# GuidoManni/BodySLAM

Hardware: AMD Instinct MI355X
Metric: frames/sec depth+pose+back-proj, 640x480 seq (higher is better)
Workload: dtype f16

## Files before the change

bodyslam_amd/_lib.py:

```python
from __future__ import annotations

import ctypes as C
import os
from typing import Optional

import torch

_HERE = os.path.dirname(os.path.abspath(__file__))
LIB_PATH = os.environ.get("BODYSLAM_HIP_LIB") or os.path.join(_HERE, "libbodyslam_hip.so")

F32, F16, BF16 = 0, 1, 2
F64 = 3
ACT_NONE, ACT_RELU, ACT_GELU, ACT_SOFTPLUS, ACT_SOFTPLUS_FAST = 0, 1, 2, 3, 4
OUT_PLAIN, OUT_SHUFFLE, OUT_QKV = 0, 1, 2

_TORCH2BS = {torch.float32: F32, torch.float16: F16, torch.bfloat16: BF16}
BS2TORCH = {F32: torch.float32, F16: torch.float16, BF16: torch.bfloat16}


class BodySlamHipError(RuntimeError):
    pass


class GemmDesc(C.Structure):
# ... 266 lines not shown
    if d.out_dtype == F32:
        per_row = [4.0, 4.0, 4.0]
    elif d.out_f8:
        per_row = [4.0, 3.0, 2.0]
    else:
        per_row = [2.0 * (2 if d.out_split_off else 1)] * 3
    full = float(d.M)
    r_planes = float(min(d.out_planes_rows, d.M)) if d.out_planes_rows else full
    r_lo = float(min(d.out_lo8_rows, d.M)) if d.out_lo8_rows else r_planes
    r_lo = min(r_lo, r_planes)
    out = d.N * (r_lo * per_row[0] + (r_planes - r_lo) * per_row[1] + (full - r_planes) * per_row[2])
    res = float(d.M) * d.N * (4 if (d.res and d.res_dtype == F32) else 0)
    return a + w + out + res


class Plan:

    def __init__(self, device=None):
        self.device = None if device is None else torch.device(device)
        self.calls = []
        self.names = []
        self.keep = []
        self.keep_descs = []
        self.marks = {}
        self.gemm_info = {}
        self.stack_info = {}
        self.events = None
        self._graph = None

    def gemm(self, name, A, W, out, **kw):
# ... 63 lines not shown
        if taps is None and self._graph is not None and not torch.cuda.is_current_stream_capturing():
            self._graph.replay()
            return
        st = torch.cuda.current_stream(self.device).cuda_stream
        if taps is None:
            for i, (fn, args) in enumerate(self.calls):
                rc = fn(*args, st)
                if rc:
                    check(rc, self.names[i])
            return
        means = taps.get("__site_means__")
        for i in range(len(self.calls) + 1):
            for (name, t, meta) in self.marks.get(i, []):
                if meta and meta[0] == "chanmean":
                    if means is not None:
                        _, off, M, lda, K = meta
                        means[name] = t.view(-1)[off: off + M * lda].view(M, lda)[:, :K].float().mean(0)
                    continue
                if means is None:
                    taps[name] = (t.clone(), meta)
            if i < len(self.calls):
                fn, args = self.calls[i]
                check(fn(*args, st), self.names[i])


_F8_ON_DEVICE = {}


def _f8_pack_device(device):
    if device is None or os.environ.get("BS_PACK_ON_HOST") == "1":
        return torch.device("cpu")
    device = torch.device(device)
# ... 340 lines not shown
```

bodyslam_amd/csrc/igemm.hip:

```cpp
#include <stdlib.h>

#include <map>
#include <mutex>
#include <utility>

#include "igemm_kernel.h"

namespace bs {

#define BS_DECL_TILE(t, cm)                                                  \
    int igemm_launch_tile##t##_f16_cm##cm(const IgemmParams&, bool, hipStream_t); \
    int igemm_launch_tile##t##_bf16_cm##cm(const IgemmParams&, bool, hipStream_t);
BS_DECL_TILE(1, 0) BS_DECL_TILE(1, 1)
BS_DECL_TILE(2, 0) BS_DECL_TILE(2, 1)
BS_DECL_TILE(3, 0) BS_DECL_TILE(3, 1)
BS_DECL_TILE(9, 0) BS_DECL_TILE(9, 1)
BS_DECL_TILE(10, 0) BS_DECL_TILE(11, 0)
BS_DECL_TILE(9s8, 0) BS_DECL_TILE(9s8, 1)
#undef BS_DECL_TILE

static int auto_tile(int M, int N, int K, int tile, bool conv) {
    if (tile != 0) return tile;
    if (N <= 32) return 3;
    if (N <= 64) return 2;
// ... 11 lines not shown
        default: BM = 128; BN = 128; break;
    }
}

static int launch_tile(IgemmParams& p, int dtype, bool conv, int tile, hipStream_t st) {
    int BM, BN;
    tile_dims(tile, BM, BN);
    p.ntm = cdiv(p.M - p.m_begin, BM);
    p.ntn = cdiv(p.N, BN);
    static const int strip_env = diag_env("BS_GEMM_STRIP") ? atoi(diag_env("BS_GEMM_STRIP")) : -1;
    const bool qkv = p.out_mode == BS_OUT_QKV;
    p.strip = conv ? 0 : (strip_env >= 0 ? strip_env : ((BM == 256 && BN == 256 && !qkv && p.ntn >= 8) ? 4 : 0));
    const int cm = (p.f8_stages > 0 || p.out_f8 || p.res_f8) ? 1 : 0;
    const bool h = dtype == BS_F16;
    const bool sched8 = tile == 9 && !(p.ablate & 32);
#define BS_TILE(t, c) (h ? igemm_launch_tile##t##_f16_cm##c(p, conv, st) : igemm_launch_tile##t##_bf16_cm##c(p, conv, st))
    switch (tile * 10 + cm) {
        case 10: return BS_TILE(1, 0);
        case 11: return BS_TILE(1, 1);
        case 20: return BS_TILE(2, 0);
        case 21: return BS_TILE(2, 1);
        case 30: return BS_TILE(3, 0);
        case 31: return BS_TILE(3, 1);
        case 90: return sched8 ? BS_TILE(9s8, 0) : BS_TILE(9, 0);
        case 91: return sched8 ? BS_TILE(9s8, 1) : BS_TILE(9, 1);
        case 100: return BS_TILE(10, 0);
        case 110: return BS_TILE(11, 0);
#undef BS_TILE
        default: set_error("bs_gemm: tile %d is not built for correction mode %d (tiles 1, 2, 3, 9, 10, 11)", tile, cm); return BS_ERR_INVALID;
    }
// ... 79 lines not shown
    BS_REQUIRE(d->lda % 8 == 0, "bs_gemm: lda=%d must be a multiple of 8 (16-byte rows)", d->lda);
    BS_REQUIRE(d->out_dtype == BS_F32 || d->out_dtype == d->dtype, "bs_gemm: out_dtype must be f32 or the operand dtype");
    BS_REQUIRE(!d->res || d->res_dtype == BS_F32 || d->res_dtype == d->dtype, "bs_gemm: res_dtype must be f32 or the operand dtype");
    IgemmParams p{};
    p.A = d->A; p.W = d->W; p.zero = zero_page();
    p.a_bytes = d->conv ? (long long)(d->M / (d->Hout > 0 && d->Wout > 0 ? d->Hout * d->Wout : 1)) * d->Hin * d->Win * d->lda * 2
                        : ((long long)(d->M - 1) * d->lda + (d->K + d->f8_seg / 2 - d->seg1)) * 2;
    BS_REQUIRE((long long)d->N * (d->K + d->f8_seg / 2) * 2 < 0x7FFFFFF0ll, "bs_gemm: weight matrix too large for one descriptor");
    p.M = d->M; p.N = d->N; p.K = d->K + d->f8_seg / 2; p.lda = d->lda;
    p.f8_seg = d->f8_seg;
    p.f8_sa0 = d->f8_scales & 0xff; p.f8_sb0 = (d->f8_scales >> 8) & 0xff; p.f8_sa1 = (d->f8_scales >> 16) & 0xff; p.f8_sb1 = d->f8_scales >> 24;
    p.out_f8 = d->out_f8;
    p.res_f8 = d->res_f8;
    BS_REQUIRE(!d->res_f8 || (d->res && d->res_dtype == d->dtype && d->res_split_off == 0 && d->ldr >= 2 * d->N && d->N % 8 == 0), "bs_gemm: res_f8 needs a 16-bit residual in (hi16 | hi8 | lo8) rows, ldr >= 2N");
    BS_REQUIRE(d->f8_seg >= 0 && d->f8_seg % 256 == 0, "bs_gemm: f8_seg=%d must be a multiple of 256 (two halves of whole 128-byte stages)", d->f8_seg);
    BS_REQUIRE(d->f8_seg == 0 || (d->seg1 == 0 && !d->relu_a), "bs_gemm: the FP8 segment excludes seg1 and relu_a");
    p.f8_stages = d->f8_seg / 128;
    BS_REQUIRE(d->out_f8 == 0 || (d->out_dtype == d->dtype && d->ldo % 8 == 0 &&
                                  ((d->out_mode == BS_OUT_PLAIN && d->out_split_off == d->N && d->N % 8 == 0) ||
                                   (d->out_mode == BS_OUT_SHUFFLE && d->out_split_off == d->shuffle_cout && d->shuffle_cout % 8 == 0))),
               "bs_gemm: out_f8 needs a plain / shuffle 16-bit output with out_split_off = channels, channels %% 8 == 0");
    p.Hin = d->Hin; p.Win = d->Win; p.Cin = d->Cin; p.Hout = d->Hout; p.Wout = d->Wout;
    p.KH = d->KH; p.KW = d->KW; p.stride = d->stride; p.pad_h = d->pad_h; p.pad_w = d->pad_w;
    if (d->conv) {
        BS_REQUIRE(d->Cin > 0 && d->Cin % 64 == 0, "bs_gemm: conv Cin=%d must be a multiple of 64", d->Cin);
        BS_REQUIRE(d->K == d->KH * d->KW * (d->Cin + d->seg1), "bs_gemm: conv K=%d != KH*KW*(Cin+seg1)", d->K);
        BS_REQUIRE(d->Hout > 0 && d->Wout > 0 && d->M % (d->Hout * d->Wout) == 0, "bs_gemm: conv M=%d not a multiple of Hout*Wout", d->M);
        BS_REQUIRE(d->stride > 0 && d->lda >= d->Cin, "bs_gemm: bad conv stride/lda");
        BS_REQUIRE(d->KH > 0 && d->KW > 0 && d->KH * d->KW <= 32, "bs_gemm: conv window %dx%d: at most 32 taps", d->KH, d->KW);
        BS_REQUIRE((long long)d->Hin * d->Win * d->lda * 2 * 4 < 0x7FFFFFF0ll, "bs_gemm: image too large for the 2 GiB tile window");
        p.tiles_per_tap = d->Cin / 64;
// ... 74 lines not shown
```

bodyslam_amd/csrc/igemm_kernel.h:

```cpp
#pragma once
#include <type_traits>

#include "common.h"

namespace bs {

struct IgemmParams {
    const void* A;
    const void* W;
    const void* zero;
    long long a_bytes;
    int M, N, K, lda;
    int Hin, Win, Cin, Hout, Wout, KH, KW, stride, pad_h, pad_w;
    int tiles_per_tap;
    int cin1;
    int split_off;
    int res_split_off;
    int relu_a;
    const float* bias;
    int bias_group_rows;
    int act;
    const float* scale;
    const void* res;
    const void* res2;
// ... 19 lines not shown
    int res_f8;
    int out_f8;
    int out2_relu;
    int out_lo8_rows;
    int f8_skip_from;
    int out_planes_rows;
    const float* bias2;
    int bias2_row0, bias2_group_rows;
    int strip;
    int ablate;
};

template <typename T>
__device__ __forceinline__ typename T16<T>::v8 relu8(typename T16<T>::v8 x) {
    typedef short s16x8 __attribute__((ext_vector_type(8)));
    s16x8 b = __builtin_bit_cast(s16x8, x);
    s16x8 neg = b >> 15;
    b = b & ~neg;
    return __builtin_bit_cast(typename T16<T>::v8, b);
}

template <typename T>
__device__ __forceinline__ void store4(void* base, int64_t off, int out_dtype, const float (&y)[4], int split_off = 0) {
    if (split_off > 0) {
        typename T16<T>::v4 h, l;
#pragma unroll
        for (int e = 0; e < 4; ++e) {
            h[e] = T16<T>::from_f32(y[e]);
            l[e] = T16<T>::from_f32(y[e] - T16<T>::to_f32(h[e]));
        }
        *reinterpret_cast<typename T16<T>::v4*>(reinterpret_cast<T*>(base) + off) = h;
        *reinterpret_cast<typename T16<T>::v4*>(reinterpret_cast<T*>(base) + off + split_off) = l;
        return;
    }
// ... 88 lines not shown
}

constexpr int NW_CHECK(int a, int b) { return a * b; }

template <int N>
__device__ __forceinline__ void wait_vmcnt() {
    asm volatile("s_waitcnt vmcnt(%0)" ::"n"(N) : "memory");
}

template <typename T, int BM, int BN, int WM, int WN, int BK, int STAGES, int MODE, bool PP = false, int CM = 0, int SCHED = 0>
__global__ __launch_bounds__(WM* WN * 64, 2) void igemm_kernel(const IgemmParams p) {
#if defined(__HIP_DEVICE_COMPILE__)
    constexpr bool CONV = MODE != 0;
    constexpr bool RELU_A = MODE == 2;
    constexpr bool F8 = CM != 0;
    constexpr int NT = WM * WN * 64;
    constexpr int ROWB = BK * 2;
    constexpr int LPR = ROWB / 16;
    constexpr int RPR = NT / LPR;
    constexpr int RPW = 64 / LPR;
    constexpr int RA = BM / RPR, RB = BN / RPR;
    static_assert(BK == 64 || BK == 32, "BK");
    static_assert(BM % RPR == 0 && BN % RPR == 0, "tile rows must be a multiple of the DMA round");
    constexpr int GL = RA + RB;
    static_assert(GL * (STAGES - 1) <= 63, "vmcnt range");
    constexpr int TM = BM / WM, TN = BN / WN;
    constexpr int FM = TM / 16, FN = TN / 16;
    static_assert(TM % 16 == 0 && TN % 16 == 0, "wave tile must be a multiple of 16");
    constexpr int A_BYTES = BM * ROWB, B_BYTES = BN * ROWB, STAGE = A_BYTES + B_BYTES;
    constexpr int LDS_BYTES = STAGES * STAGE;
// ... 221 lines not shown
                    for (int jj = 0; jj < 2; ++jj)
                        acc[ah * 4 + i][bh * 2 + jj] = __builtin_amdgcn_mfma_scale_f32_16x16x128_f8f6f4(op8(bf[bh][jj][0], bf[bh][jj][1]), a8,
                                                                                                        acc[ah * 4 + i][bh * 2 + jj], 0, 0, 0, scb, 0, sca);
                }
            } else {
#pragma unroll
                for (int kk = 0; kk < 2; ++kk)
#pragma unroll
                    for (int i = 0; i < 4; ++i)
#pragma unroll
                        for (int jj = 0; jj < 2; ++jj)
                            acc[ah * 4 + i][bh * 2 + jj] = T16<T>::mfma16(bf[bh][jj][kk], af[i][kk], acc[ah * 4 + i][bh * 2 + jj]);
            }
            __builtin_amdgcn_s_setprio(0);
        };
        auto relu_a = [&]() {
            if constexpr (RELU_A) {
#pragma unroll
                for (int i = 0; i < 4; ++i)
#pragma unroll
                    for (int kk = 0; kk < 2; ++kk) af[i][kk] = relu8<T>(af[i][kk]);
            }
        };
        auto tile = [&](int t, auto f8_tag, auto steady_tag) {
            constexpr bool F8S = decltype(f8_tag)::value == 1;
            constexpr bool STEADY = decltype(steady_tag)::value == 1;
            const int left = nt - 1 - t;
            const char* sa = smem + cbuf * STAGE;
            const char* sb = sa + A_BYTES;
            if constexpr (F8S) {
                const bool second = t >= nt16 + ((nt_all - nt16) >> 1);
                sca = (second ? p.f8_sa1 : p.f8_sa0) * 0x01010101;
                scb = (second ? p.f8_sb1 : p.f8_sb0) * 0x01010101;
            }
            read_w(sb, H0{});
            __builtin_amdgcn_sched_barrier(0);
            read_a(sa, 0);
            if ((STEADY || left >= 1) && dma) stage_piece(cbuf ^ 1, PW1{});
            if (STEADY || left >= 1) wait_vmcnt<8>();
            else wait_vmcnt<2>();
            phase_barrier();
            relu_a();
            multiply(f8_tag, H0{}, H0{});
            phase_barrier();
            read_w(sb, H1{});
            if (STEADY || left >= 1) {
                if (dma) stage_piece(cbuf ^ 1, PA1{});
                stage_advance();
                wait_vmcnt<8>();
            } else {
                wait_vmcnt<0>();
            }
            phase_barrier();
            multiply(f8_tag, H0{}, H1{});
            phase_barrier();
            read_a(sa, 1);
            if ((STEADY || left >= 2) && dma) stage_piece(cbuf, PA0{});
            phase_barrier();
            relu_a();
            multiply(f8_tag, H1{}, H1{});
            phase_barrier();
            if ((STEADY || left >= 2) && dma) stage_piece(cbuf, PW0{});
            if (STEADY || left >= 2) wait_vmcnt<8>();
            else if (left == 1) wait_vmcnt<4>();
            phase_barrier();
            multiply(f8_tag, H1{}, H0{});
            phase_barrier();
            cbuf ^= 1;
        };
        stage_piece(0, PA0{});
        stage_piece(0, PW0{});
        stage_piece(0, PW1{});
        stage_piece(0, PA1{});
        stage_advance();
// ... 1 lines not shown
            stage_piece(1, PA0{});
            stage_piece(1, PW0{});
            wait_vmcnt<8>();
        } else {
            wait_vmcnt<4>();
        }
        __builtin_amdgcn_s_waitcnt(0xc07f);
        phase_barrier();
        if (wm == 1) phase_barrier();
        using S16 = std::integral_constant<int, 0>;
        using S8 = std::integral_constant<int, 1>;
        int t = 0;
        const int n16 = nt16 < nt ? nt16 : nt;
        for (; t < n16 && t < nt - 2; ++t) tile(t, S16{}, std::integral_constant<int, 1>{});
        for (; t < n16; ++t) tile(t, S16{}, std::integral_constant<int, 0>{});
        if constexpr (F8 && !RELU_A) {
            for (; t < nt - 2; ++t) tile(t, S8{}, std::integral_constant<int, 1>{});
            for (; t < nt; ++t) tile(t, S8{}, std::integral_constant<int, 0>{});
        }
        if (wm == 0) phase_barrier();
    } else if constexpr (!PP) {
#pragma unroll
        for (int s = 0; s < STAGES - 1; ++s)
            if (s < nt) stage(s);
        int cbuf = 0, sbuf = STAGES - 1;
        v8 af[FM], bf[FN];
        auto iteration = [&](int t, auto f8_tag) {
            constexpr bool F8S = decltype(f8_tag)::value == 1;
            const int younger = nt - 1 - t;
            if (STAGES >= 4 && younger >= 2) wait_vmcnt<(STAGES >= 4 ? 2 : 0) * GL>();
            else if (STAGES >= 3 && younger >= 1) wait_vmcnt<(STAGES >= 3 ? 1 : 0) * GL>();
// ... 7 lines not shown
                typedef int i32x4 __attribute__((ext_vector_type(4)));
                typedef int i32x8 __attribute__((ext_vector_type(8)));
                const bool second = t >= nt16 + ((nt_all - nt16) >> 1);
                const int sca = (second ? p.f8_sa1 : p.f8_sa0) * 0x01010101, scb = (second ? p.f8_sb1 : p.f8_sb0) * 0x01010101;
                auto ld8 = [&](const char* base) {
                    const i32x4 lo = *reinterpret_cast<const i32x4*>(base + koff0);
                    const i32x4 hi = *reinterpret_cast<const i32x4*>(base + koff1);
                    return __builtin_shufflevector(lo, hi, 0, 1, 2, 3, 4, 5, 6, 7);
                };
                i32x8 b8[FN];
#pragma unroll
                for (int j = 0; j < FN; ++j) b8[j] = ld8(sb + b_base + j * 16 * ROWB);
                __builtin_amdgcn_s_setprio(1);
#pragma unroll
                for (int i = 0; i < FM; ++i) {
                    const i32x8 a8 = ld8(sa + a_base + i * 16 * ROWB);
#pragma unroll
                    for (int j = 0; j < FN; ++j)
                        acc[i][j] = __builtin_amdgcn_mfma_scale_f32_16x16x128_f8f6f4(b8[j], a8, acc[i][j], 0, 0, 0, scb, 0, sca);
                }
                __builtin_amdgcn_s_setprio(0);
            } else {
#pragma unroll
                for (int kk = 0; kk < BK / 32; ++kk) {
                    const int ko = kk ? koff1 : koff0;
                    if (!(p.ablate & 2) || t == 0) {
#pragma unroll
                        for (int i = 0; i < FM; ++i) {
                            af[i] = *reinterpret_cast<const v8*>(sa + a_base + i * 16 * ROWB + ko);
                            if (RELU_A) af[i] = relu8<T>(af[i]);
                        }
// ... 2 lines not shown
                    }
                    __builtin_amdgcn_s_setprio(1);
#pragma unroll
                    for (int i = 0; i < FM; ++i)
#pragma unroll
                        for (int j = 0; j < FN; ++j) acc[i][j] = T16<T>::mfma16(bf[j], af[i], acc[i][j]);
                    __builtin_amdgcn_s_setprio(0);
                }
            }
            cbuf = cbuf + 1 == STAGES ? 0 : cbuf + 1;
            sbuf = sbuf + 1 == STAGES ? 0 : sbuf + 1;
        };
        int t = 0;
        __builtin_amdgcn_s_waitcnt(0xc07f);
        for (; t < nt16; ++t) iteration(t, std::integral_constant<int, 0>{});
        if constexpr (F8 && BK == 64 && !RELU_A) {
            for (; t < nt; ++t) iteration(t, std::integral_constant<int, 1>{});
        }
    } else {
        static_assert(BK == 32 && STAGES == 4 && WM == 2 && NW_CHECK(WM, WN) == 8, "ping-pong variant: 256x256x32, 8 waves");
        const int grp = wm;
        v8 af[FM], bf[FN];
        auto load_frags = [&](int buf) {
            const char* sa = smem + buf * STAGE;
            const char* sb = sa + A_BYTES;
#pragma unroll
            for (int i = 0; i < FM; ++i) {
                af[i] = *reinterpret_cast<const v8*>(sa + a_base + i * 16 * ROWB + koff0);
                if (RELU_A) af[i] = relu8<T>(af[i]);
            }
#pragma unroll
// ... 42 lines not shown
                if (issued < last) { ++issued; stage(issued & 3); }
                load_frags(nbuf);
            }
            buf = nbuf;
        }
        if (grp == 0) phase_barrier();
    }

#define BS_FRESH_LANE                                                                                                       \
    int lane;                                                                                                               \
    asm volatile("v_mbcnt_lo_u32_b32 %0, -1, 0\n\tv_mbcnt_hi_u32_b32 %0, -1, %0" : "=v"(lane));                             \
    const int frow = lane & 15, fq = lane >> 4;                                                                             \
    (void)frow; (void)fq;
    {
    const int n_wave = tn * BN + wn * TN;
    const bool v_tile = (p.out_mode == BS_OUT_QKV) && (tn * BN >= 2 * p.qkv_hidden);
    if (p.ablate & 4) {
        if (acc[0][0][0] == 12345.678f) reinterpret_cast<float*>(p.out)[0] = 1.f;
        return;
    }
    int g2 = -1;
    bool b2_rows = false;
    if (p.bias2) {
        const int lo = m0 - p.bias2_row0, hi = (m0 + BM < p.M ? m0 + BM : p.M) - 1 - p.bias2_row0;
        if (hi >= 0) {
            if (lo >= 0 && lo / p.bias2_group_rows == hi / p.bias2_group_rows) g2 = lo / p.bias2_group_rows;
            else b2_rows = true;
        }
    }
    if (!v_tile) {
// ... 121 lines not shown
                                    add_lo8<T>(y, p.res2, orow * p.ldr, p.N, n0j[j]);
                                }
                            }
                        }
                    }
                }
#pragma unroll
                for (int jp = 0; jp < FN / 2; ++jp) {
                    float (&y8)[8] = yall[jp];
                    const int j0 = jp * 2, j1 = j0 + 1;
                    if (n0j[j0] >= p.N) continue;
                    void* dst = (p.out_mode == BS_OUT_QKV && which[j0] == 1) ? p.out2 : p.out;
                    const int so = p.out_mode != BS_OUT_QKV ? p.split_off : p.qkv_lo_off;
                    if (F8 && p.out_f8) {
                        const int nloc = p.out_mode == BS_OUT_SHUFFLE ? n0j[j0] % p.shuffle_cout : n0j[j0];
                        store8_f8<T>(dst, roff + coff[j0] - nloc, nloc, so, y8, p.out_f8 & 0xff, (p.out_f8 >> 8) & 0xff);
                    } else if (wide_ok && n0j[j1] < p.N && coff[j1] == coff[j0] + 4 && which[j1] == which[j0]) {
                        store8<T>(dst, roff + coff[j0], p.out_dtype, y8, so);
                    } else {
                        const float(&ya)[4] = *reinterpret_cast<const float(*)[4]>(y8);
                        store4<T>(dst, roff + coff[j0], p.out_dtype, ya, so);
                        if (n0j[j1] < p.N) {
                            const float(&yb)[4] = *reinterpret_cast<const float(*)[4]>(y8 + 4);
                            void* dst1 = (p.out_mode == BS_OUT_QKV && which[j1] == 1) ? p.out2 : p.out;
                            store4<T>(dst1, roff + coff[j1], p.out_dtype, yb, so);
                        }
                    }
                }
            }
        };
        const bool plain_full = p.out_mode == BS_OUT_PLAIN && !p.out_group_rows && p.bias && !p.bias_group_rows && p.N % BN == 0 &&
// ... 191 lines not shown
                            const f32x4 v = acc[i][2 * jp + h] + bj[2 * jp + h];
                            const f32x2_ g0 = gelu_erf2(f32x2_{v[0], v[1]}), g1 = gelu_erf2(f32x2_{v[2], v[3]});
                            y8[4 * h] = g0[0]; y8[4 * h + 1] = g0[1]; y8[4 * h + 2] = g1[0]; y8[4 * h + 3] = g1[1];
                        }
                        if (planes) {
                            store8_f8<T>(p.out, (int64_t)m * p.ldo, n_wave + jp * 32 + fq * 8, p.split_off, y8, p.out_f8 & 0xff, (p.out_f8 >> 8) & 0xff, lo);
                        } else {
                            typename T16<T>::v8 h;
#pragma unroll
                            for (int e = 0; e < 8; ++e) h[e] = T16<T>::from_f32(y8[e]);
                            *reinterpret_cast<typename T16<T>::v8*>(reinterpret_cast<T*>(p.out) + (int64_t)m * p.ldo + n_wave + jp * 32 + fq * 8) = h;
                        }
                    }
                }
                return;
            }
        }
        if (F8 && p.out_mode == BS_OUT_QKV && p.qkv_hidden % BN == 0 && p.act == BS_ACT_NONE && !p.res && p.bias && !p.bias_group_rows && !b2_rows &&
            p.out_dtype != BS_F32 && !(p.ablate & 16)) {
            BS_FRESH_LANE
            const int part = (tn * BN) / p.qkv_hidden;
            T* dst = reinterpret_cast<T*>(part == 1 ? p.out2 : p.out);
            const float qs = part == 0 ? p.q_scale : 1.0f;
            f32x4 bj[FN], sj[FN];
            int64_t coff[FN / 2];
#pragma unroll
            for (int j = 0; j < FN; ++j) {
                const int n0 = n_wave + (j >> 1) * 32 + fq * 8 + (j & 1) * 4;
                bj[j] = *reinterpret_cast<const f32x4*>(p.bias + n0);
                if (g2 >= 0) bj[j] += *reinterpret_cast<const f32x4*>(p.bias2 + (int64_t)g2 * p.N + n0);
// ... 271 lines not shown
    BS_MAX_DYNAMIC_LDS(reinterpret_cast<const void*>(k), smem);
    hipLaunchKernelGGL(k, grid, block, smem, st, p);
    BS_CHECK_LAUNCH();
    return BS_OK;
}

template <typename T, int BM, int BN, int WM, int WN, int BK, int STAGES, bool PP, int CM, int SCHED = 0>
inline int launch_cm(const IgemmParams& p, bool conv, hipStream_t st) {
    if constexpr (CM == 0) {
        if (!conv) return launch_mode<T, BM, BN, WM, WN, BK, STAGES, 0, PP, 0, SCHED>(p, st);
        if (p.relu_a) return launch_mode<T, BM, BN, WM, WN, BK, STAGES, 2, PP, 0, SCHED>(p, st);
        return launch_mode<T, BM, BN, WM, WN, BK, STAGES, 1, PP, 0, SCHED>(p, st);
    } else {
        static_assert(BK == 64 && !PP, "the correction instantiations are built for the BK = 64 ring tiles");
        if (!conv) return launch_mode<T, BM, BN, WM, WN, BK, STAGES, 0, PP, CM, SCHED>(p, st);
        return launch_mode<T, BM, BN, WM, WN, BK, STAGES, 1, PP, CM, SCHED>(p, st);
    }
}

}
```

bodyslam_amd/zoedepth.py:

```python
from __future__ import annotations

import math
import os
import warnings
import dataclasses
from dataclasses import dataclass
from typing import Dict, Optional, Sequence, Tuple

import numpy as np
import torch
import torch.nn.functional as F

from . import _lib as L
from .calibration import DEFAULT_POLICY, NECK_RELHEAD_WONLY, CalibrationPolicy, Scope, choose, finish_report, saving_gflop, worst

LOG2E = 1.4426950408889634


@dataclass
class ZoeConfig:
    hidden: int = 1024
    layers: int = 24
    heads: int = 16
    intermediate: int = 4096
# ... 656 lines not shown
        self.site_flops: Dict[str, float] = {}
        self.plan = L.Plan(eng.dev)
        self.pool = _Pool(eng.dev)
        self.use_tab = wp == 32 and hp <= 40
        self.grouped = grouped = self.use_tab
        self.CP = CP = (NB + 255) // 256 * 256 if grouped else 0
        self.MT = CP + NB * T0 if grouped else NB * S
        self.TOK = ("tokens_grouped" if grouped else "tokens", NB, S, c.hidden, CP)
        self.acc = acc = eng.acc
        self.m2 = 2 if acc else 1
        self.np3 = 3 if acc else 1
        self.nf8 = nf8 = eng.neck_f8
        self.NSP = (32 if nf8 else 16) if acc else 0
        self.RZ = 1 | ((4 if nf8 else 2) if acc else 0)
        self.attn_corr = bool(acc and eng.attn_mode == "corr" and self.use_tab and hp % 2 == 0)

        x = self._embed()
        taps16 = self._backbone(x)
        feats, fshape = self._reassemble(taps16)
        bins, emb = self._bins_seed(feats[3], *fshape[3])
        fused, pj_low = self._fusion(feats, fshape)
        last = self._relative_head(*fused[3])
        levels = self._levels_fused if self._projector_level_fits(fused, pj_low) else self._levels_four
        bins, Eh, ph_, pw_ = levels(fused, pj_low, bins, emb, *fshape[3])
        self._depth(last, Eh, bins, ph_, pw_)

    def e16(self, *s):
        return self.pool.alloc(s, self.eng.dtype)

    def e32(self, *s):
# ... 21 lines not shown

    def f8kw(self, wkey):
        return dict(f8_scales=self.f8_scales(wkey), f8_wonly_from=-1 if self.eng.neck_site_wonly(wkey) else 0,
                    f8_skip_from=-1 if self.eng.neck_site_plain(wkey) else 0)

    def okw(self, Cout, out_pairs, out8):
        if not (self.acc and out_pairs):
            return dict(ldo=Cout, out_split_off=0)
        return dict(ldo=Cout * self.m2, out_split_off=Cout, out_f8=self.F8O if (self.nf8 and out8) else None)

    def lo8_rows(self, *consumer_wkeys):
        return 256 if (self.acc and self.nf8 and all(k_ in self.eng.f8s and self.eng.neck_site_wonly(k_) for k_ in consumer_wkeys)) else 0

    def hi8_rows(self, *consumer_wkeys):
        return 256 if (self.acc and self.nf8 and all(k_ in self.eng.f8s and self.eng.neck_site_plain(k_) for k_ in consumer_wkeys)) else 0

    def bgemm(self, name, A, wkey, out, M, N, K, **kw):
        eng, P, w, acc, grouped, CP, NB, T0 = self.eng, self.plan, self.w, self.acc, self.grouped, self.CP, self.NB, self.T0
        f8s, mode = eng.f8s, eng.mode_of(wkey)

        def f8gemm(f8_seg, scales, **f8):
            P.gemm(name, A, w[wkey], out, M=M, N=N, K=K, lda=2 * K, f8_seg=f8_seg, f8_scales=scales, precision_passes=1, **f8, **kw)

        if acc and grouped and wkey in f8s and wkey[0] == "l":
            P.mark("in:" + wkey, A, ("chanmean", CP * 2 * K, NB * T0, 2 * K, K))
        if acc and wkey in eng.single_keys:
            P.gemm(name, A, w[wkey], out, M=M, N=N, K=K, lda=K, precision_passes=1, **kw)
        elif acc and wkey in f8s and mode == "w":
            f8gemm(K, self.f8_scales(wkey, lo_plane=False))
        elif acc and wkey in f8s and mode == "wstat" and grouped and wkey in eng.backbone_bias_corr:
# ... 9 lines not shown
            wonly = CP if (mode == "wcls" and grouped) else 0
            f8gemm(2 * K, self.f8_scales(wkey), f8_wonly_from=wonly)
        else:
            P.gemm(name, A, w[wkey], out, M=M, N=N, K=K * self.np3, lda=K * self.m2, seg1=K if acc else 0, precision_passes=self.np3, **kw)

    def nplain(self, name, A, wkey, out, M, N, K, shuffle=None, out_pairs=True, **kw):
        eng, P, w, acc = self.eng, self.plan, self.w, self.acc
        out8 = kw.pop("out8", True)
        ok = self.okw(shuffle[1] if shuffle else N, out_pairs, out8)
        if "ldo" in kw:
            ok["ldo"] = kw.pop("ldo")
        if "split_off" in kw:
            ok["out_split_off"] = kw.pop("split_off")
        if not out_pairs:
            ok = dict(ldo=ok["ldo"], out_split_off=0)
        if acc and wkey in eng.f8s:
            self.site_flops[wkey] = self.site_flops.get(wkey, 0.0) + 2.0 * M * N * K
            lda_ = kw.pop("lda", 2 * K)
            P.mark("in:" + wkey, A, ("chanmean", kw.get("a_offset", 0), M, lda_, K))
            if not kw.get("bias_group_rows"):
                kw["bias"] = eng.site_bias(wkey, kw.get("bias"))
            P.gemm(name, A, w[wkey], out, M=M, N=N, K=K, lda=lda_, f8_seg=2 * K, shuffle=shuffle,
                   precision_passes=1, **ok, **self.f8kw(wkey), **kw)
        else:
            ok.pop("out_f8", None)
            P.gemm(name, A, w[wkey], out, M=M, N=N, K=K * self.np3, lda=kw.pop("lda", K * self.m2), seg1=K if acc else 0,
                   shuffle=shuffle, precision_passes=self.np3, **ok, **kw)

    def nconv(self, name, A, wkey, out, hh, ww, Ci, Co, stride=1, **kw):
        eng, P, w, acc, NB, m2, np3 = self.eng, self.plan, self.w, self.acc, self.NB, self.m2, self.np3
        use8 = acc and wkey in eng.f8s
        g_ = L.conv_geom(hh, ww, Ci if use8 else Ci * m2, 3, 3, stride, 1)
        ho, wo = g_[3], g_[4]
        has_res = "res" in kw
        if use8:
            self.site_flops[wkey] = self.site_flops.get(wkey, 0.0) + 2.0 * NB * ho * wo * Co * 9 * Ci
            P.mark("in:" + wkey, A, ("chanmean", 0, NB * hh * ww, 2 * Ci, Ci))
            kw["bias"] = eng.site_bias(wkey, kw.get("bias"))
            P.gemm(name, A, w[wkey], out, M=NB * ho * wo, N=Co, K=9 * Ci, lda=2 * Ci, conv=g_, f8_seg=2 * Ci, ldo=2 * Co,
                   ldr=2 * Co if has_res else 0, res_f8=has_res, out_split_off=Co, out_f8=self.F8O, precision_passes=1, **self.f8kw(wkey), **kw)
        else:
            if has_res and acc:
                kw["res_split_off"] = Co
            P.gemm(name, A, w[wkey], out, M=NB * ho * wo, N=Co, K=9 * Ci * np3, lda=Ci * m2, conv=g_, seg1=Ci if acc else 0,
                   ldo=Co * m2, ldr=Co * m2 if has_res else 0, out_split_off=Co if acc else 0, precision_passes=np3, **kw)
        return ho, wo

    def _embed(self):
        c, w, P, NB, T0, S, CP, dev = self.c, self.w, self.plan, self.NB, self.T0, self.S, self.CP, self.eng.dev
        B, H, W, Hd = self.B, self.H, self.W, c.hidden
        PK = 3 * c.patch * c.patch
        self.frames = torch.empty(B, H, W, 3, device=dev, dtype=torch.uint8)
        patches = self.e16(NB * T0, PK * self.m2)
        x = torch.zeros(self.MT, Hd, device=dev, dtype=torch.float32)
        P.add("preprocess", "bs_preprocess_patches", self.frames, patches, B, H, W, self.nh, self.nw, int(self.flip), L.dt(patches) | self.fmt("pe.w"))
        if self.grouped:
# ... 52 lines not shown
        return taps16

    def _reassemble(self, taps16):
        c, w, P, eng, NB, T0, S, CP, hp, wp = self.c, self.w, self.plan, self.eng, self.NB, self.T0, self.S, self.CP, self.hp, self.wp
        acc, grouped, m2, np3, nf8, Hd = self.acc, self.grouped, self.m2, self.np3, self.nf8, c.hidden
        e16, free, nplain, nconv = self.e16, self.pool.free, self.nplain, self.nconv
        feats, fshape = [], []
        cb = self.e32(NB, Hd)
        r16 = e16(NB * T0, Hd * m2)
        for i, ch in enumerate(c.neck_hidden):
            t16 = taps16[i]
            nplain(f"ro{i}.cls", t16, f"ro{i}.w_cls", cb, NB, Hd, Hd, out_pairs=False, lda=(1 if grouped else S) * Hd * m2,
                   bias=eng.site_bias(f"ro{i}.w_tok", w[f"ro{i}.b"]))
            if grouped:
                nplain(f"ro{i}.tok", t16, f"ro{i}.w_tok", r16, NB * T0, Hd, Hd, a_offset=CP * Hd * m2, bias=cb, bias_group_rows=T0,
                       act=L.ACT_GELU)
            elif acc and f"ro{i}.w_tok" in eng.f8s:
                P.gemm(f"ro{i}.tok", t16, w[f"ro{i}.w_tok"], r16, M=NB * T0, N=Hd, K=Hd, lda=2 * Hd, conv=(1, S, Hd, 1, T0, 1, 1, 1, 0, -1),
                       f8_seg=2 * Hd, bias=cb, bias_group_rows=T0, act=L.ACT_GELU, ldo=2 * Hd, out_split_off=Hd, out_f8=self.F8O if nf8 else None,
                       precision_passes=1, **self.f8kw(f"ro{i}.w_tok"))
            else:
                P.gemm(f"ro{i}.tok", t16, w[f"ro{i}.w_tok"], r16, M=NB * T0, N=Hd, K=Hd * np3, lda=Hd * m2, conv=(1, S, Hd * m2, 1, T0, 1, 1, 1, 0, -1),
                       seg1=Hd if acc else 0, bias=cb, bias_group_rows=T0, act=L.ACT_GELU, ldo=Hd * m2, out_split_off=Hd if acc else 0,
                       precision_passes=np3)
            pr = e16(NB * T0, ch * m2)
            nplain(f"ra{i}.proj", r16, f"ra{i}.proj.w", pr, NB * T0, ch, Hd, bias=w[f"ra{i}.proj.b"])
            if i == 0 or i == 1:
                s_ = 4 if i == 0 else 2
                up = e16(NB, hp * s_, wp * s_, ch * m2)
                nplain(f"ra{i}.up", pr, f"ra{i}.up.w", up, NB * T0, s_ * s_ * ch, ch, shuffle=(s_, ch, hp, wp), bias=w[f"ra{i}.up.b"])
                free(pr)
                fh, fw, src = hp * s_, wp * s_, up
            elif i == 2:
                fh, fw, src = hp, wp, pr
            else:
                fh, fw = (hp + 2 - 3) // 2 + 1, (wp + 2 - 3) // 2 + 1
                src = e16(NB, fh, fw, ch * m2)
                nconv(f"ra{i}.down", pr, f"ra{i}.down.w", src, hp, wp, ch, ch, stride=2, bias=w[f"ra{i}.down.b"])
                free(pr)
            P.mark(f"reassemble{i}", src, ("nhwc", NB, fh, fw, ch, self.mfmt()))
            f16_ = e16(NB, fh, fw, c.fusion * m2)
            nconv(f"nc{i}", src, f"nc{i}.w", f16_, fh, fw, ch, c.fusion)
            free(src)
            P.mark(f"neckconv{i}", f16_, ("nhwc", NB, fh, fw, c.fusion, self.mfmt()))
            feats.append(f16_)
            fshape.append((fh, fw))
        free(r16, cb)
        return feats, fshape

    def _bins_seed(self, bott, bh_, bw_):
        c, w, P, NB, acc, m2, np3, dev = self.c, self.w, self.plan, self.NB, self.acc, self.m2, self.np3, self.eng.dev
        e16, e32 = self.e16, self.e32
        Mb = NB * bh_ * bw_
        xb = e16(Mb, c.bottleneck * m2)
        self.nplain("mh.conv2", bott, "mh.conv2.w", xb, Mb, c.bottleneck, c.bottleneck, bias=w["mh.conv2.b"], out8=False)
# ... 38 lines not shown
            P.gemm(f"rt{l}.o", at16, w[f"rt{l}.o.w"], tmp32, M=NB * St, N=D, K=D, lda=D, bias=w[f"rt{l}.o.b"], res=e32b, ldr=D)
            P.add(f"rt{l}.n1", "bs_layernorm", tmp32, w[f"rt{l}.n1.g"], w[f"rt{l}.n1.b"], e16b, e32b, NB * St, D, 1e-5, L.dt(e16b))
            P.gemm(f"rt{l}.l1", e16b, w[f"rt{l}.l1.w"], h16, M=NB * St, N=c.pt_inter, K=D, lda=D, bias=w[f"rt{l}.l1.b"], act=L.ACT_RELU)
            P.gemm(f"rt{l}.l2", h16, w[f"rt{l}.l2.w"], tmp32, M=NB * St, N=D, K=c.pt_inter, lda=c.pt_inter, bias=w[f"rt{l}.l2.b"], res=e32b, ldr=D)
            P.add(f"rt{l}.n2", "bs_layernorm", tmp32, w[f"rt{l}.n2.g"], w[f"rt{l}.n2.b"], e16b, e32b, NB * St, D, 1e-5, L.dt(e16b))
        c1 = e16(NB, D)
        P.gemm("cl.l1", e16b, w["cl.l1.w"], c1, M=NB, N=D, K=D, lda=St * D, bias=w["cl.l1.b"], act=L.ACT_RELU)
        P.gemm("cl.l2", c1, w["cl.l2.w"], self.logits, M=NB, N=4, K=D, lda=D, bias=w["cl.l2.b"])
        P.add("route", "bs_route_argmax", self.logits, 4, self.route, NB)
        P.mark("logits", self.logits, ("raw",))

    def res_unit(self, name, xin, hh, ww, other=None):
        w, P, NB, Fc, nf8, e16, free, nconv = self.w, self.plan, self.NB, self.c.fusion, self.nf8, self.e16, self.pool.free, self.nconv
        t = e16(NB, hh, ww, Fc * self.m2)
        y = e16(NB, hh, ww, Fc * self.m2)
        if self.acc:
            xr = e16(NB, hh, ww, Fc * self.m2)
            P.add(name + ".relu", "bs_relu_split", xin, xr, NB * hh * ww, Fc, L.dt(xr) | (32 if nf8 else 0) | (64 if self.lo8_rows(name + ".c1.w") else 0) | (128 if self.hi8_rows(name + ".c1.w") else 0))
            nconv(name + ".c1", xr, name + ".c1.w", t, hh, ww, Fc, Fc, bias=w[name + ".c1.b"], act=L.ACT_RELU, out_lo8_rows=self.lo8_rows(name + ".c2.w"),
                  out_planes_rows=self.hi8_rows(name + ".c2.w"))
            free(xr)
        else:
            nconv(name + ".c1", xin, name + ".c1.w", t, hh, ww, Fc, Fc, relu_a=True, bias=w[name + ".c1.b"], act=L.ACT_RELU)
        nconv(name + ".c2", t, name + ".c2.w", y, hh, ww, Fc, Fc, bias=w[name + ".c2.b"], res=xin, res2=other)
        free(t)
        return y

    def _fusion(self, feats, fshape):
        w, P, eng, NB, m2, Fc, PM = self.w, self.plan, self.eng, self.NB, self.m2, self.c.fusion, self.c.proj_mlp
        e16, free, nplain = self.e16, self.pool.free, self.nplain
        rh_in = "rh.projection.w" if eng.add_projection else "rh.conv1.w"
# ... 20 lines not shown
            pj_low.append((z, fh, fw))
            fused = e16(NB, 2 * fh, 2 * fw, Fc * m2)
            nolo = bool(li == 3 and self.lo8_rows(rh_in))
            nopl = bool(nolo and self.hi8_rows(rh_in))
            P.add(f"fu{li}.up", "bs_resize_bilinear_nhwc", lowp, fused, NB, fh, fw, Fc, 2 * fh, 2 * fw, self.RZ | (8 if nolo else 0) | (16 if nopl else 0), L.dt(fused))
            free(lowp)
            P.mark(f"fused{li}", fused, ("nhwc", NB, 2 * fh, 2 * fw, Fc, 3 if nolo else self.mfmt()))
            fused_list.append((fused, 2 * fh, 2 * fw))
        return fused_list, pj_low

    def _relative_head(self, f3, h3, w3):
        c, w, P, eng, NB, acc, m2, nf8, Fc = self.c, self.w, self.plan, self.eng, self.NB, self.acc, self.m2, self.nf8, self.c.fusion
        e16, free, nconv = self.e16, self.pool.free, self.nconv
        if eng.add_projection:
            rp = e16(NB, h3, w3, Fc * m2)
            nconv("rh.projection", f3, "rh.projection.w", rp, h3, w3, Fc, Fc, bias=w["rh.projection.b"], act=L.ACT_RELU, out_lo8_rows=self.lo8_rows("rh.conv1.w"))
            free(f3)
        else:
            rp = f3
        r1 = e16(NB, h3, w3, (Fc // 2) * m2)
        nconv("rh.conv1", rp, "rh.conv1.w", r1, h3, w3, Fc, Fc // 2, bias=w["rh.conv1.b"], out_lo8_rows=self.lo8_rows("rh.conv2.w"))
        free(rp)
        fused_up = (os.environ.get("BS_UPCONV_FUSED", "1") != "0" and Fc // 2 == 128 and c.rel_features == 32
                    and ((not acc) or (nf8 and "rh.conv2.w" in eng.f8s)))
        if fused_up:
            last = e16(NB, 2 * h3, 2 * w3, c.rel_features * m2)
            if acc:
                umode, usc = (1 if eng.neck_site_wonly("rh.conv2.w") else 2), self.f8_scales("rh.conv2.w")
                self.site_flops["rh.conv2.w"] = 2.0 * NB * h3 * w3 * 9 * c.rel_features * (Fc // 2)
            else:
                umode, usc = 0, (127, 127, 127, 127)
# ... 126 lines not shown
```

Baseline: 503.1.

## Fuse ReLU into FP8 conv A-loads and trim unused output planes in neck

Measured after the change: 507.4 (median of 6 runs). Within noise of the previous version (+0.8%).

```diff
diff --git a/bodyslam_amd/_lib.py b/bodyslam_amd/_lib.py
--- a/bodyslam_amd/_lib.py
+++ b/bodyslam_amd/_lib.py
@@ -304,6 +304,14 @@
     return a + w + out + res
 
 
+def chanmean(t: torch.Tensor, meta) -> torch.Tensor:
+    off, M, lda, K = meta[1:5]
+    a = t.view(-1)[off: off + M * lda].view(M, lda)[:, :K].float()
+    if len(meta) > 5 and meta[5]:
+        a = a.clamp_min(0.0)
+    return a.mean(0)
+
+
 class Plan:
 
     def __init__(self, device=None):
@@ -397,8 +405,7 @@
             for (name, t, meta) in self.marks.get(i, []):
                 if meta and meta[0] == "chanmean":
                     if means is not None:
-                        _, off, M, lda, K = meta
-                        means[name] = t.view(-1)[off: off + M * lda].view(M, lda)[:, :K].float().mean(0)
+                        means[name] = chanmean(t, meta)
                     continue
                 if means is None:
                     taps[name] = (t.clone(), meta)
diff --git a/bodyslam_amd/csrc/igemm.hip b/bodyslam_amd/csrc/igemm.hip
--- a/bodyslam_amd/csrc/igemm.hip
+++ b/bodyslam_amd/csrc/igemm.hip
@@ -49,6 +49,10 @@
     const int cm = (p.f8_stages > 0 || p.out_f8 || p.res_f8) ? 1 : 0;
     const bool h = dtype == BS_F16;
     const bool sched8 = tile == 9 && !(p.ablate & 32);
+    if (tile == 9 && !sched8 && cm && conv && p.relu_a && p.f8_stages > 0 && p.f8_skip_from != -1) {
+        set_error("bs_gemm: relu_a beside FP8 stages is not built for tile 9's one-barrier loop (ablation bit 32)");
+        return BS_ERR_INVALID;
+    }
 #define BS_TILE(t, c) (h ? igemm_launch_tile##t##_f16_cm##c(p, conv, st) : igemm_launch_tile##t##_bf16_cm##c(p, conv, st))
     switch (tile * 10 + cm) {
         case 10: return BS_TILE(1, 0);
@@ -158,7 +162,9 @@
     p.res_f8 = d->res_f8;
     BS_REQUIRE(!d->res_f8 || (d->res && d->res_dtype == d->dtype && d->res_split_off == 0 && d->ldr >= 2 * d->N && d->N % 8 == 0), "bs_gemm: res_f8 needs a 16-bit residual in (hi16 | hi8 | lo8) rows, ldr >= 2N");
     BS_REQUIRE(d->f8_seg >= 0 && d->f8_seg % 256 == 0, "bs_gemm: f8_seg=%d must be a multiple of 256 (two halves of whole 128-byte stages)", d->f8_seg);
-    BS_REQUIRE(d->f8_seg == 0 || (d->seg1 == 0 && !d->relu_a), "bs_gemm: the FP8 segment excludes seg1 and relu_a");
+    BS_REQUIRE(d->f8_seg == 0 || d->seg1 == 0, "bs_gemm: the FP8 segment excludes seg1");
+    BS_REQUIRE(d->f8_seg == 0 || !d->relu_a || d->f8_skip_from == -1 || d->f8_wonly_from == -1,
+               "bs_gemm: relu_a beside an FP8 segment needs f8_skip_from = -1 or f8_wonly_from = -1 (no tile may run the A_lo8 x W_hi8 stage)");
     p.f8_stages = d->f8_seg / 128;
     BS_REQUIRE(d->out_f8 == 0 || (d->out_dtype == d->dtype && d->ldo % 8 == 0 &&
                                   ((d->out_mode == BS_OUT_PLAIN && d->out_split_off == d->N && d->N % 8 == 0) ||
diff --git a/bodyslam_amd/csrc/igemm_kernel.h b/bodyslam_amd/csrc/igemm_kernel.h
--- a/bodyslam_amd/csrc/igemm_kernel.h
+++ b/bodyslam_amd/csrc/igemm_kernel.h
@@ -57,10 +57,16 @@
 template <typename T>
 __device__ __forceinline__ typename T16<T>::v8 relu8(typename T16<T>::v8 x) {
     typedef short s16x8 __attribute__((ext_vector_type(8)));
-    s16x8 b = __builtin_bit_cast(s16x8, x);
-    s16x8 neg = b >> 15;
-    b = b & ~neg;
+    const s16x8 b = __builtin_elementwise_max(__builtin_bit_cast(s16x8, x), s16x8{0, 0, 0, 0, 0, 0, 0, 0});
     return __builtin_bit_cast(typename T16<T>::v8, b);
+}
+
+__device__ __forceinline__ int relu_f8x4(int x) {
+    int t;
+    asm volatile("v_lshrrev_b32 %1, 7, %0\n\tv_and_b32 %1, 0x01010101, %1\n\tv_lshl_or_b32 %1, %1, 1, %1\n\tv_lshl_or_b32 %1, %1, 2, %1\n\t"
+                 "v_lshl_or_b32 %1, %1, 4, %1\n\tv_bfi_b32 %0, %1, 0, %0"
+                 : "+v"(x), "=&v"(t));
+    return x;
 }
 
 template <typename T>
@@ -179,6 +185,7 @@
     constexpr bool CONV = MODE != 0;
     constexpr bool RELU_A = MODE == 2;
     constexpr bool F8 = CM != 0;
+    constexpr bool F8_STAGES = F8 && !(RELU_A && BM == 256 && SCHED == 0);
     constexpr int NT = WM * WN * 64;
     constexpr int ROWB = BK * 2;
     constexpr int LPR = ROWB / 16;
@@ -430,12 +437,22 @@
             }
             __builtin_amdgcn_s_setprio(0);
         };
-        auto relu_a = [&]() {
+        auto relu_a = [&](auto f8_tag) {
             if constexpr (RELU_A) {
+                typedef int i32x4 __attribute__((ext_vector_type(4)));
 #pragma unroll
                 for (int i = 0; i < 4; ++i)
 #pragma unroll
-                    for (int kk = 0; kk < 2; ++kk) af[i][kk] = relu8<T>(af[i][kk]);
+                    for (int kk = 0; kk < 2; ++kk) {
+                        if constexpr (decltype(f8_tag)::value == 1) {
+                            i32x4 b = __builtin_bit_cast(i32x4, af[i][kk]);
+#pragma unroll
+                            for (int e = 0; e < 4; ++e) b[e] = relu_f8x4(b[e]);
+                            af[i][kk] = __builtin_bit_cast(v8, b);
+                        } else {
+                            af[i][kk] = relu8<T>(af[i][kk]);
+                        }
+                    }
             }
         };
         auto tile = [&](int t, auto f8_tag, auto steady_tag) {
@@ -456,7 +473,7 @@
             if (STEADY || left >= 1) wait_vmcnt<8>();
             else wait_vmcnt<2>();
             phase_barrier();
-            relu_a();
+            relu_a(f8_tag);
             multiply(f8_tag, H0{}, H0{});
             phase_barrier();
             read_w(sb, H1{});
@@ -473,7 +490,7 @@
             read_a(sa, 1);
             if ((STEADY || left >= 2) && dma) stage_piece(cbuf, PA0{});
             phase_barrier();
-            relu_a();
+            relu_a(f8_tag);
             multiply(f8_tag, H1{}, H1{});
             phase_barrier();
             if ((STEADY || left >= 2) && dma) stage_piece(cbuf, PW0{});
@@ -505,7 +522,7 @@
         const int n16 = nt16 < nt ? nt16 : nt;
         for (; t < n16 && t < nt - 2; ++t) tile(t, S16{}, std::integral_constant<int, 1>{});
         for (; t < n16; ++t) tile(t, S16{}, std::integral_constant<int, 0>{});
-        if constexpr (F8 && !RELU_A) {
+        if constexpr (F8) {
             for (; t < nt - 2; ++t) tile(t, S8{}, std::integral_constant<int, 1>{});
             for (; t < nt; ++t) tile(t, S8{}, std::integral_constant<int, 0>{});
         }
@@ -543,7 +560,11 @@
                 __builtin_amdgcn_s_setprio(1);
 #pragma unroll
                 for (int i = 0; i < FM; ++i) {
-                    const i32x8 a8 = ld8(sa + a_base + i * 16 * ROWB);
+                    i32x8 a8 = ld8(sa + a_base + i * 16 * ROWB);
+                    if constexpr (RELU_A) {
+#pragma unroll
+                        for (int e = 0; e < 8; ++e) a8[e] = relu_f8x4(a8[e]);
+                    }
 #pragma unroll
                     for (int j = 0; j < FN; ++j)
                         acc[i][j] = __builtin_amdgcn_mfma_scale_f32_16x16x128_f8f6f4(b8[j], a8, acc[i][j], 0, 0, 0, scb, 0, sca);
@@ -576,7 +597,7 @@
         int t = 0;
         __builtin_amdgcn_s_waitcnt(0xc07f);
         for (; t < nt16; ++t) iteration(t, std::integral_constant<int, 0>{});
-        if constexpr (F8 && BK == 64 && !RELU_A) {
+        if constexpr (F8_STAGES && BK == 64) {
             for (; t < nt; ++t) iteration(t, std::integral_constant<int, 1>{});
         }
     } else {
@@ -649,6 +670,8 @@
     (void)frow; (void)fq;
     {
     const int n_wave = tn * BN + wn * TN;
+    const bool hi_plane = !(F8 && p.out_planes_rows > 0 && m0 >= p.out_planes_rows);
+    const bool lo_plane = hi_plane && !(F8 && p.out_lo8_rows > 0 && m0 >= p.out_lo8_rows);
     const bool v_tile = (p.out_mode == BS_OUT_QKV) && (tn * BN >= 2 * p.qkv_hidden);
     if (p.ablate & 4) {
         if (acc[0][0][0] == 12345.678f) reinterpret_cast<float*>(p.out)[0] = 1.f;
@@ -800,7 +823,7 @@
                     const int so = p.out_mode != BS_OUT_QKV ? p.split_off : p.qkv_lo_off;
                     if (F8 && p.out_f8) {
                         const int nloc = p.out_mode == BS_OUT_SHUFFLE ? n0j[j0] % p.shuffle_cout : n0j[j0];
-                        store8_f8<T>(dst, roff + coff[j0] - nloc, nloc, so, y8, p.out_f8 & 0xff, (p.out_f8 >> 8) & 0xff);
+                        store8_f8<T>(dst, roff + coff[j0] - nloc, nloc, so, y8, p.out_f8 & 0xff, (p.out_f8 >> 8) & 0xff, lo_plane, hi_plane);
                     } else if (wide_ok && n0j[j1] < p.N && coff[j1] == coff[j0] + 4 && which[j1] == which[j0]) {
                         store8<T>(dst, roff + coff[j0], p.out_dtype, y8, so);
                     } else {
@@ -1022,6 +1045,83 @@
                     }
                 }
                 return;
+            }
+            if constexpr (TN == 64 && LDS_BYTES >= WM * WN * TM * 128) {
+                const bool shuf = p.out_mode == BS_OUT_SHUFFLE;
+                if (p.out_f8 && p.out_planes_rows > 0 && m0 >= p.out_planes_rows && !(p.ablate & (16 | 1024)) && p.ldo % 8 == 0 && !p.scale && !p.res &&
+                    !p.bias2 && p.out_dtype != BS_F32 && p.act <= BS_ACT_GELU &&
+                    (shuf ? p.shuffle_cout % BN == 0 : (p.out_mode == BS_OUT_PLAIN && !p.out_group_rows && p.N % BN == 0))) {
+                    auto staged = [&](auto act_tag) {
+                        constexpr int ACT = decltype(act_tag)::value;
+                        BS_FRESH_LANE
+                        typedef unsigned u32x4_ __attribute__((ext_vector_type(4)));
+                        f32x4 bj[FN];
+#pragma unroll
+                        for (int j = 0; j < FN; ++j) {
+                            const int n0 = n_wave + (j >> 1) * 32 + fq * 8 + (j & 1) * 4;
+                            bj[j] = (p.bias && !p.bias_group_rows) ? *reinterpret_cast<const f32x4*>(p.bias + n0) : f32x4{0.f, 0.f, 0.f, 0.f};
+                        }
+                        __syncthreads();
+                        char* sw = smem + wave * (TM * 128);
+                        const int s7 = frow & 7;
+                        const int wb0 = frow * 128 + ((fq ^ s7) << 4), wb1 = frow * 128 + (((4 + fq) ^ s7) << 4);
+#pragma unroll
+                        for (int i = 0; i < FM; ++i) {
+                            int mb = m0 + wm * TM + i * 16 + frow;
+                            mb = mb < p.M ? mb : p.M - 1;
+                            const float* brow = (p.bias && p.bias_group_rows) ? p.bias + (int64_t)(mb / p.bias_group_rows) * p.N + n_wave + fq * 8 : nullptr;
+#pragma unroll
+                            for (int jp = 0; jp < FN / 2; ++jp) {
+                                typename T16<T>::v8 h8v;
+#pragma unroll
+                                for (int h = 0; h < 2; ++h) {
+                                    const f32x4 b = brow ? *reinterpret_cast<const f32x4*>(brow + jp * 32 + h * 4) : bj[2 * jp + h];
+                                    float y[4];
+#pragma unroll
+                                    for (int e = 0; e < 4; ++e) y[e] = acc[i][2 * jp + h][e] + b[e];
+                                    if (ACT == BS_ACT_GELU) {
+                                        const f32x2_ g0 = gelu_erf2(f32x2_{y[0], y[1]}), g1 = gelu_erf2(f32x2_{y[2], y[3]});
+                                        y[0] = g0[0]; y[1] = g0[1]; y[2] = g1[0]; y[3] = g1[1];
+                                    }
+#pragma unroll
+                                    for (int e = 0; e < 4; ++e) {
+                                        if (ACT == BS_ACT_RELU) y[e] = fmaxf(y[e], 0.0f);
+                                        h8v[4 * h + e] = T16<T>::from_f32(y[e]);
+                                    }
+                                }
+                                *reinterpret_cast<typename T16<T>::v8*>(sw + (jp ? wb1 : wb0) + i * 2048) = h8v;
+                            }
+                        }
+                        __builtin_amdgcn_fence(__ATOMIC_RELEASE, "wavefront");
+                        __builtin_amdgcn_wave_barrier();
+                        const int rr = lane >> 3, pc = lane & 7;
+                        const int rb = rr * 128 + ((pc ^ rr) << 4);
+                        int64_t cofs = n_wave + pc * 8;
+                        if (shuf) {
+                            const int s = p.shuffle_s;
+                            const int tap = (tn * BN) / p.shuffle_cout, ky = tap / s, kx = tap - ky * s;
+                            cofs = ((int64_t)ky * (p.Wout * s) + kx) * p.ldo + (n_wave - tap * p.shuffle_cout) + pc * 8;
+                        }
+                        T* outp = reinterpret_cast<T*>(p.out) + cofs;
+#pragma unroll
+                        for (int it = 0; it < TM / 8; ++it) {
+                            const int m = m0 + wm * TM + it * 8 + rr;
+                            if (m >= p.M) continue;
+                            int64_t roff = (int64_t)m * p.ldo;
+                            if (shuf) {
+                                const int hw = p.Hout * p.Wout, s = p.shuffle_s;
+                                const int ob = m / hw, rem = m - ob * hw;
+                                const int oy = rem / p.Wout, ox = rem - oy * p.Wout;
+                                roff = (((int64_t)(ob * p.Hout + oy) * s) * (p.Wout * s) + ox * s) * p.ldo;
+                            }
+                            *reinterpret_cast<u32x4_*>(outp + roff) = *reinterpret_cast<const u32x4_*>(sw + rb + it * 1024);
+                        }
+                    };
+                    if (p.act == BS_ACT_GELU) staged(std::integral_constant<int, BS_ACT_GELU>{});
+                    else if (p.act == BS_ACT_RELU) staged(std::integral_constant<int, BS_ACT_RELU>{});
+                    else staged(std::integral_constant<int, BS_ACT_NONE>{});
+                    return;
+                }
             }
         }
         if (F8 && p.out_mode == BS_OUT_QKV && p.qkv_hidden % BN == 0 && p.act == BS_ACT_NONE && !p.res && p.bias && !p.bias_group_rows && !b2_rows &&
@@ -1323,6 +1423,7 @@
     } else {
         static_assert(BK == 64 && !PP, "the correction instantiations are built for the BK = 64 ring tiles");
         if (!conv) return launch_mode<T, BM, BN, WM, WN, BK, STAGES, 0, PP, CM, SCHED>(p, st);
+        if (p.relu_a) return launch_mode<T, BM, BN, WM, WN, BK, STAGES, 2, PP, CM, SCHED>(p, st);
         return launch_mode<T, BM, BN, WM, WN, BK, STAGES, 1, PP, CM, SCHED>(p, st);
     }
 }
diff --git a/bodyslam_amd/zoedepth.py b/bodyslam_amd/zoedepth.py
--- a/bodyslam_amd/zoedepth.py
+++ b/bodyslam_amd/zoedepth.py
@@ -694,6 +694,8 @@
         self.NSP = (32 if nf8 else 16) if acc else 0
         self.RZ = 1 | ((4 if nf8 else 2) if acc else 0)
         self.attn_corr = bool(acc and eng.attn_mode == "corr" and self.use_tab and hp % 2 == 0)
+        lean = os.environ.get("BS_NECK_LEAN", "1")
+        self.lean_relu, self.lean_planes = lean in ("1", "relu"), lean in ("1", "planes")
 
         x = self._embed()
         taps16 = self._backbone(x)
@@ -745,6 +747,14 @@
 
     def hi8_rows(self, *consumer_wkeys):
         return 256 if (self.acc and self.nf8 and all(k_ in self.eng.f8s and self.eng.neck_site_plain(k_) for k_ in consumer_wkeys)) else 0
+
+    def lean_rows(self, *consumer_wkeys):
+        if not self.lean_planes:
+            return {}
+        return dict(out_lo8_rows=self.lo8_rows(*consumer_wkeys), out_planes_rows=self.hi8_rows(*consumer_wkeys))
+
+    def lean_fmt(self, *consumer_wkeys):
+        return 3 if (self.lean_planes and self.lo8_rows(*consumer_wkeys)) else self.mfmt()
 
     def bgemm(self, name, A, wkey, out, M, N, K, **kw):
         eng, P, w, acc, grouped, CP, NB, T0 = self.eng, self.plan, self.w, self.acc, self.grouped, self.CP, self.NB, self.T0
@@ -784,6 +794,9 @@
             ok["out_split_off"] = kw.pop("split_off")
         if not out_pairs:
             ok = dict(ldo=ok["ldo"], out_split_off=0)
+        if not (acc and wkey in eng.f8s and ok.get("out_f8")):
+            kw.pop("out_lo8_rows", None)
+            kw.pop("out_planes_rows", None)
         if acc and wkey in eng.f8s:
             self.site_flops[wkey] = self.site_flops.get(wkey, 0.0) + 2.0 * M * N * K
             lda_ = kw.pop("lda", 2 * K)
@@ -805,11 +818,13 @@
         has_res = "res" in kw
         if use8:
             self.site_flops[wkey] = self.site_flops.get(wkey, 0.0) + 2.0 * NB * ho * wo * Co * 9 * Ci
-            P.mark("in:" + wkey, A, ("chanmean", 0, NB * hh * ww, 2 * Ci, Ci))
+            P.mark("in:" + wkey, A, ("chanmean", 0, NB * hh * ww, 2 * Ci, Ci, bool(kw.get("relu_a"))))
             kw["bias"] = eng.site_bias(wkey, kw.get("bias"))
             P.gemm(name, A, w[wkey], out, M=NB * ho * wo, N=Co, K=9 * Ci, lda=2 * Ci, conv=g_, f8_seg=2 * Ci, ldo=2 * Co,
                    ldr=2 * Co if has_res else 0, res_f8=has_res, out_split_off=Co, out_f8=self.F8O, precision_passes=1, **self.f8kw(wkey), **kw)
         else:
+            kw.pop("out_lo8_rows", None)
+            kw.pop("out_planes_rows", None)
             if has_res and acc:
                 kw["res_split_off"] = Co
             P.gemm(name, A, w[wkey], out, M=NB * ho * wo, N=Co, K=9 * Ci * np3, lda=Ci * m2, conv=g_, seg1=Ci if acc else 0,
@@ -892,21 +907,23 @@
                    bias=eng.site_bias(f"ro{i}.w_tok", w[f"ro{i}.b"]))
             if grouped:
                 nplain(f"ro{i}.tok", t16, f"ro{i}.w_tok", r16, NB * T0, Hd, Hd, a_offset=CP * Hd * m2, bias=cb, bias_group_rows=T0,
-                       act=L.ACT_GELU)
+                       act=L.ACT_GELU, **self.lean_rows(f"ra{i}.proj.w"))
             elif acc and f"ro{i}.w_tok" in eng.f8s:
                 P.gemm(f"ro{i}.tok", t16, w[f"ro{i}.w_tok"], r16, M=NB * T0, N=Hd, K=Hd, lda=2 * Hd, conv=(1, S, Hd, 1, T0, 1, 1, 1, 0, -1),
                        f8_seg=2 * Hd, bias=cb, bias_group_rows=T0, act=L.ACT_GELU, ldo=2 * Hd, out_split_off=Hd, out_f8=self.F8O if nf8 else None,
-                       precision_passes=1, **self.f8kw(f"ro{i}.w_tok"))
+                       precision_passes=1, **self.f8kw(f"ro{i}.w_tok"), **(self.lean_rows(f"ra{i}.proj.w") if nf8 else {}))
             else:
                 P.gemm(f"ro{i}.tok", t16, w[f"ro{i}.w_tok"], r16, M=NB * T0, N=Hd, K=Hd * np3, lda=Hd * m2, conv=(1, S, Hd * m2, 1, T0, 1, 1, 1, 0, -1),
                        seg1=Hd if acc else 0, bias=cb, bias_group_rows=T0, act=L.ACT_GELU, ldo=Hd * m2, out_split_off=Hd if acc else 0,
                        precision_passes=np3)
             pr = e16(NB * T0, ch * m2)
-            nplain(f"ra{i}.proj", r16, f"ra{i}.proj.w", pr, NB * T0, ch, Hd, bias=w[f"ra{i}.proj.b"])
+            nplain(f"ra{i}.proj", r16, f"ra{i}.proj.w", pr, NB * T0, ch, Hd, bias=w[f"ra{i}.proj.b"],
+                   **self.lean_rows((f"ra{i}.up.w", f"ra{i}.up.w", f"nc{i}.w", f"ra{i}.down.w")[i]))
             if i == 0 or i == 1:
                 s_ = 4 if i == 0 else 2
                 up = e16(NB, hp * s_, wp * s_, ch * m2)
-                nplain(f"ra{i}.up", pr, f"ra{i}.up.w", up, NB * T0, s_ * s_ * ch, ch, shuffle=(s_, ch, hp, wp), bias=w[f"ra{i}.up.b"])
+                nplain(f"ra{i}.up", pr, f"ra{i}.up.w", up, NB * T0, s_ * s_ * ch, ch, shuffle=(s_, ch, hp, wp), bias=w[f"ra{i}.up.b"],
+                       **self.lean_rows(f"nc{i}.w"))
                 free(pr)
                 fh, fw, src = hp * s_, wp * s_, up
             elif i == 2:
@@ -914,9 +931,9 @@
             else:
                 fh, fw = (hp + 2 - 3) // 2 + 1, (wp + 2 - 3) // 2 + 1
                 src = e16(NB, fh, fw, ch * m2)
-                nconv(f"ra{i}.down", pr, f"ra{i}.down.w", src, hp, wp, ch, ch, stride=2, bias=w[f"ra{i}.down.b"])
+                nconv(f"ra{i}.down", pr, f"ra{i}.down.w", src, hp, wp, ch, ch, stride=2, bias=w[f"ra{i}.down.b"], **self.lean_rows(f"nc{i}.w"))
                 free(pr)
-            P.mark(f"reassemble{i}", src, ("nhwc", NB, fh, fw, ch, self.mfmt()))
+            P.mark(f"reassemble{i}", src, ("nhwc", NB, fh, fw, ch, self.lean_fmt(f"nc{i}.w")))
             f16_ = e16(NB, fh, fw, c.fusion * m2)
             nconv(f"nc{i}", src, f"nc{i}.w", f16_, fh, fw, ch, c.fusion)
             free(src)
@@ -985,7 +1002,11 @@
         w, P, NB, Fc, nf8, e16, free, nconv = self.w, self.plan, self.NB, self.c.fusion, self.nf8, self.e16, self.pool.free, self.nconv
         t = e16(NB, hh, ww, Fc * self.m2)
         y = e16(NB, hh, ww, Fc * self.m2)
-        if self.acc:
+        c1 = name + ".c1.w"
+        if self.acc and nf8 and self.lean_relu and c1 in self.eng.f8s and (self.eng.neck_site_plain(c1) or self.eng.neck_site_wonly(c1)):
+            nconv(name + ".c1", xin, c1, t, hh, ww, Fc, Fc, relu_a=True, bias=w[name + ".c1.b"], act=L.ACT_RELU,
+                  out_lo8_rows=self.lo8_rows(name + ".c2.w"), out_planes_rows=self.hi8_rows(name + ".c2.w"))
+        elif self.acc:
             xr = e16(NB, hh, ww, Fc * self.m2)
             P.add(name + ".relu", "bs_relu_split", xin, xr, NB * hh * ww, Fc, L.dt(xr) | (32 if nf8 else 0) | (64 if self.lo8_rows(name + ".c1.w") else 0) | (128 if self.hi8_rows(name + ".c1.w") else 0))
             nconv(name + ".c1", xr, name + ".c1.w", t, hh, ww, Fc, Fc, bias=w[name + ".c1.b"], act=L.ACT_RELU, out_lo8_rows=self.lo8_rows(name + ".c2.w"),
@@ -1036,7 +1057,8 @@
         e16, free, nconv = self.e16, self.pool.free, self.nconv
         if eng.add_projection:
             rp = e16(NB, h3, w3, Fc * m2)
-            nconv("rh.projection", f3, "rh.projection.w", rp, h3, w3, Fc, Fc, bias=w["rh.projection.b"], act=L.ACT_RELU, out_lo8_rows=self.lo8_rows("rh.conv1.w"))
+            nconv("rh.projection", f3, "rh.projection.w", rp, h3, w3, Fc, Fc, bias=w["rh.projection.b"], act=L.ACT_RELU, out_lo8_rows=self.lo8_rows("rh.conv1.w"),
+                  out_planes_rows=self.hi8_rows("rh.conv1.w") if self.lean_planes else 0)
             free(f3)
         else:
             rp = f3
```
